# AnamarijaKic/bioinfo1

Measured on AMD Instinct MI355X. Metric: GCUPS (DP cell updates/s) at 1/2/4/8 GPUs; bit-exact score+CIGAR, higher is better.
Workload: dtype int32 semantics; packed int16 arithmetic where range-proven (fits_int16), else int32; 1 GPU; config 2: 10000 uniform 1000x1000 pairs per GPU, local, scoring 1,-1,-1, CIGAR on; pairs_per_gpu=10000, qlen=1000, tlen=1000, mode=local, cigar=True, cells_per_gpu=10000000000, cells_total=10000000000, parallelism=pairs range-split over 1 GPU(s)

## Files before the change

bioinfo1_amd/align.py:

```python
from __future__ import annotations

import ctypes as C
import enum
import os
from dataclasses import dataclass

import numpy as np

HERE = os.path.dirname(os.path.abspath(__file__))
LIB_PATH = os.path.join(HERE, "libteam_alignment.so")

TA_OK, TA_ERR_BAD_TYPE, TA_ERR_CIGAR, TA_ERR_ARG, TA_ERR_DEVICE, TA_ERR_CAPACITY, TA_ERR_RANGE, TA_ERR_UNSERVED = range(8)
TA_PLAN_INT32_ONLY, TA_PLAN_NO_FLEX, TA_PLAN_UNFUSED, TA_PLAN_WALK1, TA_PLAN_WALK2 = 1, 2, 4, 8, 16
TA_PLAN_SERIAL_PASSES, TA_PLAN_PASS_MAJOR, TA_PLAN_NO_BLK, TA_PLAN_NO_CK, TA_PLAN_CK = 32, 64, 128, 256, 512
TA_PLAN_NO_FLEX_CK = 1024


class AlignmentType(enum.IntEnum):

    global_ = 0
    local = 1
    semiGlobal = 2


class DeviceError(RuntimeError):
    pass


_lib = None


def lib() -> C.CDLL:
    global _lib
    if _lib is not None:
        return _lib
    try:
        import torch
    except ImportError:
        pass
    if not os.path.exists(LIB_PATH):
        raise ImportError(f"{LIB_PATH} missing: run `python -c 'import __graft_entry__ as g; g.build()'`")
    L = C.CDLL(LIB_PATH)
    u32p, u64p, i32p = C.POINTER(C.c_uint32), C.POINTER(C.c_uint64), C.POINTER(C.c_int32)
    L.ta_status_string.restype = C.c_char_p
    L.ta_status_string.argtypes = [C.c_int]
    L.ta_last_error.restype = C.c_char_p
    L.ta_last_error.argtypes = [C.c_void_p]
    L.ta_context_create.argtypes = [C.c_int, C.POINTER(C.c_void_p)]
    L.ta_context_destroy.argtypes = [C.c_void_p]
    L.ta_context_destroy.restype = None
    L.ta_cigar_slot_bytes.restype = C.c_uint64
    L.ta_cigar_slot_bytes.argtypes = [C.c_uint32, C.c_uint32]
    L.ta_align_batch.argtypes = [C.c_void_p, C.c_uint32, C.c_void_p, u64p, u32p, C.c_void_p, u64p, u32p, C.c_int,
                                 C.c_int, C.c_int, C.c_int, C.c_int, i32p, u32p, C.c_void_p, C.c_uint64, u64p, u32p]
    L.ta_align_batch_flags.argtypes = L.ta_align_batch.argtypes + [C.c_uint32]
    L.ta_context_release.argtypes = [C.c_void_p]
    L.ta_context_release.restype = None
    L.ta_context_held_bytes.argtypes = [C.c_void_p]
    L.ta_context_held_bytes.restype = C.c_uint64
    L.ta_set_default_device.argtypes = [C.c_int]
    L.ta_set_thread_device.argtypes = [C.c_int]
    L.ta_plan_create.argtypes = [C.c_void_p, C.c_uint32, u32p, u32p, C.c_int, C.c_int, C.c_int, C.c_int, C.c_int,
                                 C.c_uint64, C.c_uint32, C.POINTER(C.c_void_p)]
    L.ta_plan_destroy.argtypes = [C.c_void_p]
    L.ta_plan_destroy.restype = None
    for f in ("ta_plan_cigar_slots_bytes", "ta_plan_workspace_bytes"):
        getattr(L, f).restype = C.c_uint64
        getattr(L, f).argtypes = [C.c_void_p]
    L.ta_plan_chunks.restype = C.c_uint32
    L.ta_plan_chunks.argtypes = [C.c_void_p]
    L.ta_plan_dual_pairs.restype = C.c_uint32
    L.ta_plan_dual_pairs.argtypes = [C.c_void_p]
    L.ta_plan_flex_pairs.restype = C.c_uint32
    L.ta_plan_flex_pairs.argtypes = [C.c_void_p]
    L.ta_plan_fused.argtypes = [C.c_void_p]
    L.ta_plan_walk.argtypes = [C.c_void_p]
    L.ta_plan_pair_chunks.argtypes = [C.c_void_p, u32p]
    L.ta_affine_plan_pair_chunks.argtypes = [C.c_void_p, u32p]
    L.ta_plan_execute.argtypes = [C.c_void_p, C.c_void_p, C.c_void_p]
    L.ta_plan_check.argtypes = [C.c_void_p]
    L.ta_compact_cigars.argtypes = [C.c_void_p, C.c_uint32, C.c_void_p, C.c_void_p, C.c_void_p, C.c_void_p,
                                    C.c_void_p, C.c_void_p]
    L.ta_plan_execute_fill.argtypes = [C.c_void_p, C.c_void_p, C.c_void_p, C.c_uint32]
    L.ta_plan_execute_traceback.argtypes = [C.c_void_p, C.c_void_p, C.c_void_p, C.c_uint32]
    L.ta_pipeline_create.argtypes = [C.POINTER(C.c_void_p), C.c_uint32, C.POINTER(C.c_void_p)]
    L.ta_pipeline_create_affine.argtypes = L.ta_pipeline_create.argtypes
    L.ta_pipeline_step.argtypes = [C.c_void_p, C.c_void_p, C.c_void_p, C.c_void_p, u32p]
    L.ta_pipeline_destroy.argtypes = [C.c_void_p]
    L.ta_pipeline_destroy.restype = None
    L.ta_align_batch_affine.argtypes = [C.c_void_p, C.c_uint32, C.c_void_p, u64p, u32p, C.c_void_p, u64p, u32p,
                                        C.c_int, C.c_int, C.c_int, C.c_int, C.c_int, C.c_int, i32p, u32p, C.c_void_p,
                                        C.c_uint64, u64p, u32p]
    L.ta_affine_plan_create.argtypes = [C.c_void_p, C.c_uint32, u32p, u32p, C.c_int, C.c_int, C.c_int, C.c_int,
                                        C.c_int, C.c_int, C.c_uint64, C.c_uint32, C.POINTER(C.c_void_p)]
    L.ta_affine_plan_destroy.argtypes = [C.c_void_p]
    L.ta_affine_plan_destroy.restype = None
    for f in ("ta_affine_plan_cigar_slots_bytes", "ta_affine_plan_workspace_bytes"):
        getattr(L, f).restype = C.c_uint64
        getattr(L, f).argtypes = [C.c_void_p]
    L.ta_affine_plan_chunks.restype = C.c_uint32
    L.ta_affine_plan_chunks.argtypes = [C.c_void_p]
    L.ta_affine_plan_dual_pairs.restype = C.c_uint32
    L.ta_affine_plan_dual_pairs.argtypes = [C.c_void_p]
    L.ta_affine_plan_execute.argtypes = [C.c_void_p, C.c_void_p, C.c_void_p]
    L.ta_affine_plan_execute_fill.argtypes = [C.c_void_p, C.c_void_p, C.c_void_p, C.c_uint32]
    L.ta_affine_plan_execute_traceback.argtypes = [C.c_void_p, C.c_void_p, C.c_void_p, C.c_uint32]
    L.ta_affine_plan_check.argtypes = [C.c_void_p]
    L.ta_align_batch_banded.argtypes = [C.c_void_p, C.c_uint32, C.c_void_p, u64p, u32p, C.c_void_p, u64p, u32p, u32p,
                                        C.c_int, C.c_int, C.c_int, C.c_int, C.c_int, i32p, u32p, C.c_void_p,
                                        C.c_uint64, u64p, u32p]
    L.ta_banded_plan_create.argtypes = [C.c_void_p, C.c_uint32, u32p, u32p, u32p, C.c_int, C.c_int, C.c_int, C.c_int,
                                        C.c_int, C.c_uint64, C.c_uint32, C.POINTER(C.c_void_p)]
    L.ta_banded_plan_destroy.argtypes = [C.c_void_p]
    L.ta_banded_plan_destroy.restype = None
    for f in ("ta_banded_plan_cigar_slots_bytes", "ta_banded_plan_workspace_bytes", "ta_banded_plan_band_cells",
              "ta_banded_plan_swept_cells"):
        getattr(L, f).restype = C.c_uint64
        getattr(L, f).argtypes = [C.c_void_p]
    L.ta_banded_plan_chunks.restype = C.c_uint32
    L.ta_banded_plan_chunks.argtypes = [C.c_void_p]
    L.ta_banded_plan_pair_chunks.argtypes = [C.c_void_p, u32p]
    L.ta_banded_plan_execute.argtypes = [C.c_void_p, C.c_void_p, C.c_void_p]
    L.ta_banded_plan_execute_fill.argtypes = [C.c_void_p, C.c_void_p, C.c_void_p, C.c_uint32]
    L.ta_banded_plan_execute_traceback.argtypes = [C.c_void_p, C.c_void_p, C.c_void_p, C.c_uint32]
    L.ta_banded_plan_check.argtypes = [C.c_void_p]
    L.ta_banded_plan_annotate.argtypes = [C.c_void_p, C.c_void_p, C.c_void_p, C.c_void_p]
    L.ta_plan_annotate.argtypes = [C.c_void_p, C.c_void_p, C.c_void_p, C.c_void_p]
    L.ta_affine_plan_annotate.argtypes = [C.c_void_p, C.c_void_p, C.c_void_p, C.c_void_p]
    L.ta_server_create.argtypes = [C.c_int, C.c_int, C.c_uint32, C.POINTER(C.c_void_p)]
    L.ta_server_destroy.argtypes = [C.c_void_p]
    L.ta_server_destroy.restype = None
    L.ta_server_fits.argtypes = [C.c_void_p, C.c_uint32, C.c_uint32, C.c_int, C.c_int, C.c_int]
    L.ta_server_running.argtypes = [C.c_void_p]
    L.ta_server_last_times.argtypes = [C.c_void_p, C.c_uint32, C.POINTER(C.c_double)]
    L.ta_server_align.argtypes = [C.c_void_p, C.c_char_p, C.c_uint32, C.c_char_p, C.c_uint32, C.c_int, C.c_int,
                                  C.c_int, C.c_int, C.POINTER(C.c_int32), C.POINTER(C.c_uint32), C.c_void_p,
                                  C.c_uint64, C.POINTER(C.c_uint32)]
    _lib = L
    return L


ABI_SYMBOLS = [
    "ta_status_string", "ta_last_error", "ta_context_create", "ta_context_destroy", "ta_context_release",
    "ta_context_held_bytes", "ta_set_default_device", "ta_set_thread_device", "ta_current_device", "ta_device_count",
    "ta_cigar_slot_bytes", "ta_align_batch", "ta_align_batch_flags", "ta_plan_create", "ta_plan_destroy", "ta_plan_cigar_slots_bytes",
    "ta_plan_workspace_bytes", "ta_plan_chunks", "ta_plan_dual_pairs", "ta_plan_flex_pairs", "ta_plan_fused", "ta_plan_walk",
    "ta_plan_execute", "ta_plan_check", "ta_plan_execute_fill", "ta_plan_pair_chunks", "ta_affine_plan_pair_chunks", "ta_plan_execute_traceback", "ta_compact_cigars",
    "ta_affine_plan_create", "ta_affine_plan_destroy", "ta_affine_plan_cigar_slots_bytes",
    "ta_affine_plan_workspace_bytes", "ta_affine_plan_chunks", "ta_affine_plan_dual_pairs", "ta_affine_plan_execute", "ta_affine_plan_execute_fill",
    "ta_affine_plan_execute_traceback", "ta_affine_plan_check", "ta_align_batch_affine",
    "ta_server_create", "ta_server_destroy", "ta_server_fits", "ta_server_align", "ta_server_running",
    "ta_server_last_times", "ta_server_pause", "ta_server_resume",
    "ta_plan_annotate", "ta_affine_plan_annotate",
    "ta_plan_context", "ta_affine_plan_context", "ta_context_device",
    "ta_pipeline_create", "ta_pipeline_create_affine", "ta_pipeline_step", "ta_pipeline_destroy",
]
BANDED_ABI_SYMBOLS = [
    "ta_banded_plan_create", "ta_banded_plan_destroy", "ta_banded_plan_cigar_slots_bytes",
    "ta_banded_plan_workspace_bytes", "ta_banded_plan_chunks", "ta_banded_plan_pair_chunks",
    "ta_banded_plan_band_cells", "ta_banded_plan_swept_cells", "ta_banded_plan_execute",
    "ta_banded_plan_execute_fill", "ta_banded_plan_execute_traceback", "ta_banded_plan_check",
    "ta_banded_plan_annotate", "ta_align_batch_banded",
]
ABI_SYMBOLS += BANDED_ABI_SYMBOLS
TEAM_ALIGN_SYMBOL = ("_ZN4team5AlignEPKcjS1_jNS_13AlignmentTypeEiiiPNSt7__cxx1112basic_stringIcSt11char_traitsIcESaIcEEEPj")


def _check_type(type) -> int:
    t = int(type)
    if t not in (0, 1, 2):
        raise ValueError("Unknown AlignmentType provided.")
    return t


def _raise(status: int, ctx=None):
    L = lib()
    msg = L.ta_status_string(status).decode()
    if status in (TA_ERR_BAD_TYPE, TA_ERR_CIGAR, TA_ERR_RANGE):
        raise ValueError(msg)
    detail = L.ta_last_error(ctx).decode() if ctx else ""
    raise DeviceError(f"{msg}: {detail}" if detail else msg)


def _p(a, ct):
    return a.ctypes.data_as(C.POINTER(ct))


def _band_array(band, n_pairs: int) -> np.ndarray:
    if np.ndim(band) == 0:
        b = np.full(n_pairs, int(band), np.int64)
    else:
        b = np.asarray(band, np.int64).reshape(-1)
        if b.size != n_pairs:
            raise ValueError(f"band: {b.size} entries for {n_pairs} pairs")
    if b.size and (b.min() < 0 or b.max() > 0xFFFFFFFF):
        raise ValueError("band: values must be in [0, 2^32)")
    return np.ascontiguousarray(b.astype(np.uint32))


@dataclass
class BatchResult:
    scores: np.ndarray
    target_begins: np.ndarray
    cigar_offsets: np.ndarray | None
    cigar_lens: np.ndarray | None
    arena: np.ndarray | None

    def cigar(self, p: int) -> bytes | None:
        if self.arena is None:
            return None
        o = int(self.cigar_offsets[p])
        return self.arena[o : o + int(self.cigar_lens[p])].tobytes()

    def cigars(self):
        return [self.cigar(p) for p in range(len(self.scores))]


class Aligner:

    def __init__(self, device: int = 0):
        L = lib()
        h = C.c_void_p()
        r = L.ta_context_create(device, C.byref(h))
        if r != TA_OK:
            raise DeviceError(f"ta_context_create(device={device}): {L.ta_status_string(r).decode()}")
        self._h = h
        self.device = device

    def close(self):
        if getattr(self, "_h", None):
            lib().ta_context_destroy(self._h)
            self._h = None

    def __del__(self):
        try:
            self.close()
        except Exception:
            pass
# ... 316 lines not shown
            self.eqx_len = torch.zeros(self.P, dtype=torch.int32, device=self.dev)
        self._annotated_eqx = bool(eqx)
        aio = _AnnotateIO(self.info.data_ptr(), self.eqx_slots.data_ptr() if eqx else None,
                          self.eqx_start.data_ptr() if eqx else None, self.eqx_len.data_ptr() if eqx else None)
        r = self._fn("ta_plan_annotate")(self._h, C.byref(self.io), C.byref(aio), self._stream())
        if r != TA_OK:
            _raise(r, self._ctx)

    def annotation(self) -> Annotation:
        if getattr(self, "info", None) is None:
            raise RuntimeError("annotation(): no annotate() was enqueued")
        self.check()
        info = np.ascontiguousarray(self.info.cpu().numpy()).view(np.uint32).reshape(self.P, 10)
        info = info.view(PAIR_INFO_DTYPE).reshape(self.P)
        if not self._annotated_eqx:
            return Annotation(info, None, None, None)
        return Annotation(info, self.eqx_start.cpu().numpy().view(np.uint64),
                          self.eqx_len.cpu().numpy().view(np.uint32), self.eqx_slots.cpu().numpy())

    def compact_cigars(self, out=None):
        torch = self.torch
        lens = self.cigar_len.to(torch.int64)
        if out is None:
            off = torch.zeros(self.P + 1, dtype=torch.int64, device=self.dev)
            dst = torch.empty(max(self.slots_bytes, 1), dtype=torch.uint8, device=self.dev)
        else:
            dst, off = out
        torch.cumsum(lens, 0, out=off[1:])
        r = lib().ta_compact_cigars(self._ctx, self.P, self.slots.data_ptr(), self.cigar_start.data_ptr(),
                                    self.cigar_len.data_ptr(), off.data_ptr(), dst.data_ptr(), self._stream())
        if r != TA_OK:
            _raise(r, self._ctx)
        return dst, off

    def compact_buffers(self):
        torch = self.torch
        return (torch.empty(max(self.slots_bytes, 1), dtype=torch.uint8, device=self.dev),
                torch.zeros(self.P + 1, dtype=torch.int64, device=self.dev))

    def pair_chunks(self) -> np.ndarray:
        out = np.zeros(max(self.P, 1), np.uint32)
        r = self._fn("ta_plan_pair_chunks")(self._h, _p(out, C.c_uint32))
        if r != TA_OK:
            _raise(r, self._ctx)
        return out[: self.P]

    def results_at(self, indices) -> BatchResult:
        torch = self.torch
        self.check()
        idx = torch.as_tensor(np.asarray(indices, np.int64), device=self.dev)
        sc = self.score[idx].cpu().numpy()
        tb = self.target_begin[idx].cpu().numpy().view(np.uint32)
        if not self.want_cigar:
            return BatchResult(sc, tb, None, None, None)
        start = self.cigar_start[idx].cpu().numpy()
        ln = self.cigar_len[idx].cpu().numpy().view(np.uint32)
        parts, offs, o = [], np.zeros(len(ln), np.uint64), 0
        for k in range(len(ln)):
            parts.append(self.slots[int(start[k]):int(start[k]) + int(ln[k])].cpu().numpy())
            offs[k] = o
            o += int(ln[k])
        arena = np.concatenate(parts) if parts else np.zeros(1, np.uint8)
        return BatchResult(sc, tb, offs, ln, arena)

    def results(self) -> BatchResult:
        self.check()
        return _results(self)

    def close(self):
        if getattr(self, "_h", None):
            self._fn("ta_plan_destroy")(self._h)
            self._h = None

    def __del__(self):
        try:
            self.close()
        except Exception:
            pass


class DevicePipeline:

    def __init__(self, device: int, batch, type, match, mismatch, gap, want_cigar=True, depth: int = 3,
                 workspace_budget: int = 0, gap_open=None, flags: int = 0, inputs=None, first=None):
        import torch

        self.torch = torch
        self.dev = torch.device("cuda", device)
        self.aligners, self.plans, self.k = [], [], 0
        for k in range(depth):
            if k == 0 and first is not None:
                self.plans.append(first)
                continue
            al = Aligner(device)
            self.aligners.append(al)
            shared = inputs if not self.plans else (self.plans[0].qbytes, self.plans[0].qoff,
                                                    self.plans[0].tbytes, self.plans[0].toff)
            self.plans.append(DevicePlan(al, batch, type, match, mismatch, gap, want_cigar,
                                         workspace_budget=workspace_budget, gap_open=gap_open, flags=flags,
                                         inputs=shared))
        L = lib()
        handles = (C.c_void_p * len(self.plans))(*[p._h for p in self.plans])
        h = C.c_void_p()
        create = L.ta_pipeline_create_affine if self.plans[0].affine else L.ta_pipeline_create
        r = create(handles, len(self.plans), C.byref(h))
        if r != TA_OK:
            msg = L.ta_last_error(self.plans[0]._ctx).decode()
            for p in self.plans[1 if first is not None else 0:]:
                p.close()
            for al in self.aligners:
                al.close()
            if r == TA_ERR_ARG:
                raise ValueError(msg or "ta_pipeline_create: invalid argument")
            raise DeviceError(f"{L.ta_status_string(r).decode()}: {msg}")
        self._h = h

    @property
    def chunks(self):
        return self.plans[0].chunks

    def step(self, inputs=None, ready=None):
        if ready is not None and inputs is None:
            raise ValueError("DevicePipeline.step: ready without inputs (the event belongs to an upload of inputs)")
        plan = self.plans[self.k % len(self.plans)]
        if inputs is not None:
            plan.set_inputs(inputs)
        cur = self.torch.cuda.current_stream(self.dev)
        slot = C.c_uint32()
        ev = C.c_void_p(ready.cuda_event) if ready is not None else None
        r = lib().ta_pipeline_step(self._h, C.byref(plan.io), ev, C.c_void_p(cur.cuda_stream), C.byref(slot))
        if r != TA_OK:
            _raise(r, plan._ctx)
        assert self.plans[slot.value] is plan
        self.k += 1
        return plan

    def check(self):
        for p in self.plans:
            p.check()

    def close(self):
        if getattr(self, "_h", None):
            lib().ta_pipeline_destroy(self._h)
            self._h = None
        for p in self.plans:
            p.close()
        for al in self.aligners:
            al.close()


class HostBatchRunner:

    def __init__(self, aligner: Aligner, batch, type, match, mismatch, gap, want_cigar=True):
        import torch

        self.t = _check_type(type)
        self.sc = (match, mismatch, gap)
        self.want_cigar = bool(want_cigar)
        self.aligner = aligner
        self.P = P = batch.n_pairs

        def pinned(a):
            a = np.ascontiguousarray(a)
            t = torch.empty(max(a.nbytes, 1), dtype=torch.uint8, pin_memory=True)
            v = t.numpy()[: a.nbytes].view(a.dtype)
            v[...] = a.reshape(-1)
            return t, v

        self._keep = []
        for name, a in (("qb", batch.qbytes if batch.qbytes.size else np.zeros(1, np.uint8)), ("qoff", batch.qoff),
                        ("qlen", batch.qlen), ("tb", batch.tbytes if batch.tbytes.size else np.zeros(1, np.uint8)),
                        ("toff", batch.toff), ("tlen", batch.tlen), ("score", np.zeros(P, np.int32)),
                        ("tbeg", np.zeros(P, np.uint32)), ("coff", np.zeros(P, np.uint64)),
                        ("clen", np.zeros(P, np.uint32))):
            t, v = pinned(a)
            self._keep.append(t)
            setattr(self, name, v)
        cap = int((2 * (batch.qlen.astype(np.uint64) + batch.tlen.astype(np.uint64)) + 2).sum()) if P else 1
        t, self.arena = pinned(np.zeros(max(cap, 1), np.uint8))
        self._keep.append(t)
        self.cap = cap

    def run(self):
        L = lib()
        r = L.ta_align_batch(
            self.aligner.handle, self.P, self.qb.ctypes.data, _p(self.qoff, C.c_uint64), _p(self.qlen, C.c_uint32),
            self.tb.ctypes.data, _p(self.toff, C.c_uint64), _p(self.tlen, C.c_uint32), self.t, *self.sc,
            int(self.want_cigar), _p(self.score, C.c_int32), _p(self.tbeg, C.c_uint32), self.arena.ctypes.data,
            self.cap, _p(self.coff, C.c_uint64), _p(self.clen, C.c_uint32))
        if r != TA_OK:
            _raise(r, self.aligner.handle)

    def results(self) -> BatchResult:
        if not self.want_cigar:
            return BatchResult(self.score.copy(), self.tbeg.copy(), None, None, None)
        return BatchResult(self.score.copy(), self.tbeg.copy(), self.coff.copy(), self.clen.copy(), self.arena.copy())


# ... 109 lines not shown
```

bioinfo1_amd/csrc/ta_kernels.hip:

```cpp
#include <algorithm>
#include <cstdlib>

#include "ta_device.h"
#include "ta_walk2.h"
#include "ta_walk_lane.h"
#include "ta_walk_band.h"

namespace ta {
namespace {

#ifdef TA_FILL_MODE
struct PairOut {
    int score;
    uint32_t tb, gi, gj;
    uint64_t cstart;
    uint32_t clen;
};

template <int MODE>
__device__ __forceinline__ PairOut degenerate(int gap, uint32_t n, uint32_t m) {
    PairOut o{0, 0, 0, 0, 0, 0};
    if (MODE == kGlobal) {
        o.gi = n;
        o.gj = m;
// ... 722 lines not shown
                       hb = (uint32_t)rdlane((int)v, 2);
        if (seq != last) {
            __builtin_amdgcn_fence(__ATOMIC_ACQUIRE, "");
            serve_one<MODE>(sa, s, slot, seq, lane, wall_clock64(), lds);
            last = seq;
            t_hb = wall_clock64();
            continue;
        }
        if (stop) break;
        const uint64_t now = wall_clock64();
        if (hb != hb_last) {
            hb_last = hb;
            t_hb = now;
        } else if (now - t_hb > sa.hb_timeout) {
            break;
        }
        __builtin_amdgcn_s_sleep(2);
    }
}
#endif

#endif

#ifdef TA_TU_MISC
template <int MODE>
#ifndef TA_TB_WPE
#define TA_TB_WPE 8
#endif
__global__ __launch_bounds__(kBlock) __attribute__((amdgpu_waves_per_eu(TA_TB_WPE))) void traceback_kernel(TraceArgs a) {
    const int lane = threadIdx.x & 63;
    const uint32_t stride = gridDim.x * kWavesPerBlock;
    for (uint32_t widx = wave_id(); widx < a.count; widx += stride) {
        const uint32_t p = a.order ? a.order[a.begin + widx] : a.begin + widx;
        const uint32_t n = a.qlen[p], m = a.tlen[p];
        uint64_t st;
        uint32_t len;
        const WalkSeq seq{a.qbytes + a.qoff[p], a.tbytes + a.toff[p], MODE == kLocal ? a.score[p] : 0, a.match,
                          a.mismatch, a.gap};
        traceback_pair<MODE>(a.ptrs + a.ptr_off[p], n, m, a.goal_i[p], a.goal_j[p], a.slots + a.slot_off[p],
                             cigar_slot_bytes(n, m), lane, &st, &len, seq, a.blk != 0);
        if (lane == 0) {
            a.cigar_start[p] = a.slot_off[p] + st;
            a.cigar_len[p] = len;
        }
    }
}

template <int G>
__global__ __launch_bounds__(kBlock) void traceback_group_kernel(TraceArgs a) {
    const uint32_t widx = wave_id();
    if ((64u / G) * widx >= a.count) return;
    traceback_group_local<G>(a, widx, threadIdx.x & 63);
}

template <int G>
__global__ __launch_bounds__(kWave) void traceback_lane_kernel(TraceArgs a) {
    __shared__ uint32_t lds[(64 / G) * kLwGroupDw];
    traceback_lane_local<G>(a, lds, (int)threadIdx.x);
}

__global__ __launch_bounds__(kWave) __attribute__((amdgpu_waves_per_eu(1, 1))) void traceback_band_kernel(TraceArgs a) {
    __shared__ __attribute__((aligned(16))) uint8_t lds[kWave * kBwRegion + kBwStageBytes];
    const int lane = (int)threadIdx.x;
    traceback_band_local(a, lds, lane);
    if (a.fb_count) {
        const uint32_t nfb = *a.fb_count;
        for (uint32_t w = blockIdx.x; w < nfb; w += gridDim.x) {
            const uint32_t p = a.fb_order[w];
            const uint32_t n = a.qlen[p], m = a.tlen[p];
            uint64_t st;
            uint32_t len;
            const WalkSeq seq{a.qbytes + a.qoff[p], a.tbytes + a.toff[p], a.score[p], a.match, a.mismatch, a.gap};
            traceback_pair<kLocal>(a.ptrs + a.ptr_off[p], n, m, a.goal_i[p], a.goal_j[p], a.slots + a.slot_off[p],
                                   cigar_slot_bytes(n, m), lane, &st, &len, seq, true);
            if (lane == 0) {
                a.cigar_start[p] = a.slot_off[p] + st;
                a.cigar_len[p] = len;
            }
        }
    }
}

__global__ __launch_bounds__(kBlock) void format_runs_kernel(TraceArgs a) {
    const uint32_t w = wave_id();
    if (w >= a.count) return;
    format_runs(a, a.order ? a.order[a.begin + w] : a.begin + w, threadIdx.x & 63);
}

__global__ __launch_bounds__(kBlock) void compact_kernel(CompactArgs a) {
    const int lane = threadIdx.x & 63;
    const uint32_t p = wave_id();
    if (p >= a.n_pairs) return;
    const char* src = a.slots + a.cigar_start[p];
    char* dst = a.dst + a.dst_off[p];
    const uint32_t len = a.cigar_len[p];
    for (uint32_t k = (uint32_t)lane; k < len; k += 64u) dst[k] = src[k];
}

#endif

inline dim3 grid_for(uint32_t waves) { return dim3((waves + kWavesPerBlock - 1) / kWavesPerBlock); }

}

#ifdef TA_FILL_MODE
template <>
hipError_t launch_fill_mode<TA_FILL_MODE, (TA_FILL_CIGAR != 0)>(bool wide, const FillArgs& a, hipStream_t s) {
    constexpr int MODE = TA_FILL_MODE;
    constexpr bool CIGAR = TA_FILL_CIGAR != 0;
    if (!a.count) return hipSuccess;
    const dim3 g = grid_for(a.count), b(kBlock);
    if (a.count_dev && a.max_blocks) {
        const dim3 gb(std::min<uint32_t>(g.x, a.max_blocks));
        if (MODE == kLocal && wide) hipLaunchKernelGGL((fill_back_kernel<MODE, CIGAR, MODE == kLocal>), gb, b, 0, s, a);
        else hipLaunchKernelGGL((fill_back_kernel<MODE, CIGAR, false>), gb, b, 0, s, a);
        return hipGetLastError();
    }
    if (a.tasks64) {
        if (a.n_tasks) {
            const dim3 gt = grid_for(a.n_tasks);
            if (MODE == kLocal && wide) hipLaunchKernelGGL((fill_pipe_kernel<MODE, CIGAR, MODE == kLocal>), gt, b, 0, s, a);
            else hipLaunchKernelGGL((fill_pipe_kernel<MODE, CIGAR, false>), gt, b, 0, s, a);
        }
        hipLaunchKernelGGL(fill_combine_kernel<MODE>, dim3((a.count + 255) / 256), dim3(256), 0, s, a);
        return hipGetLastError();
    }
    if (MODE == kLocal && wide) hipLaunchKernelGGL((fill_kernel<MODE, CIGAR, MODE == kLocal>), g, b, 0, s, a);
    else hipLaunchKernelGGL((fill_kernel<MODE, CIGAR, false>), g, b, 0, s, a);
    return hipGetLastError();
}
#if TA_FILL_CIGAR
template <>
hipError_t launch_serve_mode<TA_FILL_MODE>(const ServeArgs& a, uint32_t slots, hipStream_t s) {
    hipLaunchKernelGGL(serve_kernel<TA_FILL_MODE>, dim3(slots), dim3(kWave), 0, s, a);
    return hipGetLastError();
}
#endif
#endif

#ifdef TA_TU_MISC
#ifndef TA_LW_G
#define TA_LW_G 16
#endif
hipError_t launch_fill(int mode, bool cigar, bool wide, const FillArgs& a, hipStream_t s) {
    switch (mode * 2 + (cigar ? 1 : 0)) {
        case 0: return launch_fill_mode<kGlobal, false>(wide, a, s);
        case 1: return launch_fill_mode<kGlobal, true>(wide, a, s);
        case 2: return launch_fill_mode<kLocal, false>(wide, a, s);
        case 3: return launch_fill_mode<kLocal, true>(wide, a, s);
        case 4: return launch_fill_mode<kSemi, false>(wide, a, s);
        case 5: return launch_fill_mode<kSemi, true>(wide, a, s);
        default: return hipErrorInvalidValue;
    }
}

hipError_t launch_dual(int mode, bool cigar, const FillArgs& a, hipStream_t s) {
    switch (mode * 2 + (cigar ? 1 : 0)) {
        case 0: return launch_dual_mode<kGlobal, false>(a, s);
        case 1: return launch_dual_mode<kGlobal, true>(a, s);
        case 2: return launch_dual_mode<kLocal, false>(a, s);
        case 3: return launch_dual_mode<kLocal, true>(a, s);
        case 4: return launch_dual_mode<kSemi, false>(a, s);
        case 5: return launch_dual_mode<kSemi, true>(a, s);
        default: return hipErrorInvalidValue;
    }
}
// ... 85 lines not shown
```

bioinfo1_amd/csrc/ta_pipeline.cpp:

```cpp
#ifndef __HIP_PLATFORM_AMD__
#define __HIP_PLATFORM_AMD__ 1
#endif
#include <hip/hip_runtime_api.h>

#include <string>
#include <vector>

#include "../../include/team_align_c.h"
#include "ta_pipeline_internal.h"

namespace {

struct Ops {
    ta_context* (*context)(const void*);
    uint32_t (*chunks)(const void*);
    int (*fill)(void*, const ta_device_io*, void*, uint32_t);
    int (*walk)(void*, const ta_device_io*, void*, uint32_t);
};

const Ops kLinear = {
    [](const void* p) { return ta_plan_context(static_cast<const ta_plan*>(p)); },
    [](const void* p) { return ta_plan_chunks(static_cast<const ta_plan*>(p)); },
    [](void* p, const ta_device_io* io, void* s, uint32_t c) {
        return ta_plan_execute_fill(static_cast<ta_plan*>(p), io, s, c);
    },
    [](void* p, const ta_device_io* io, void* s, uint32_t c) {
        return ta_plan_execute_traceback(static_cast<ta_plan*>(p), io, s, c);
    },
};

const Ops kAffine = {
    [](const void* p) { return ta_affine_plan_context(static_cast<const ta_affine_plan*>(p)); },
    [](const void* p) { return ta_affine_plan_chunks(static_cast<const ta_affine_plan*>(p)); },
    [](void* p, const ta_device_io* io, void* s, uint32_t c) {
        return ta_affine_plan_execute_fill(static_cast<ta_affine_plan*>(p), io, s, c);
    },
    [](void* p, const ta_device_io* io, void* s, uint32_t c) {
        return ta_affine_plan_execute_traceback(static_cast<ta_affine_plan*>(p), io, s, c);
    },
};

int fail(ta_context* ctx, int code, const std::string& msg) {
    ta_context_set_error(ctx, msg.c_str());
    return code;
}

#define TP_HIP(ctx, expr)                                                                     \
    do {                                                                                      \
        hipError_t e_ = (expr);                                                               \
        if (e_ != hipSuccess)                                                                 \
            return fail((ctx), TA_ERR_DEVICE, std::string(#expr) + ": " + hipGetErrorString(e_)); \
    } while (0)

}

struct ta_pipeline {
    const Ops* ops = nullptr;
    int device = 0;
    std::vector<void*> slots;
    std::vector<ta_context*> ctxs;
    std::vector<hipStream_t> fill;
    hipStream_t walk = nullptr;
    std::vector<hipEvent_t> done, walked;
    hipEvent_t start = nullptr;
    std::vector<bool> used;
    uint64_t k = 0;
    int last = -1;
};

namespace {

int create(const Ops& ops, void* const* slots, uint32_t depth, ta_pipeline** out) {
    if (!out) return TA_ERR_ARG;
    *out = nullptr;
    if (!slots || !depth || !slots[0]) return TA_ERR_ARG;
    ta_context* c0 = ops.context(slots[0]);
    if (!c0) return TA_ERR_ARG;
    if (depth < 2) return fail(c0, TA_ERR_ARG, "ta_pipeline_create: depth must be at least 2");
    for (uint32_t a = 0; a < depth; ++a) {
        ta_context* ca = slots[a] ? ops.context(slots[a]) : nullptr;
        if (!ca) return fail(c0, TA_ERR_ARG, "ta_pipeline_create: null slot");
        if (ta_context_device(ca) != ta_context_device(c0))
            return fail(c0, TA_ERR_ARG, "ta_pipeline_create: slots on different devices");
        for (uint32_t b = 0; b < a; ++b)
            if (ops.context(slots[b]) == ca)
                return fail(c0, TA_ERR_ARG, "ta_pipeline_create: two slots share a context (each needs its own workspace)");
    }
    auto* p = new ta_pipeline();
    p->ops = &ops;
    p->device = ta_context_device(c0);
    p->slots.assign(slots, slots + depth);
    for (uint32_t a = 0; a < depth; ++a) p->ctxs.push_back(ops.context(slots[a]));
    p->fill.assign(depth, nullptr);
    p->done.assign(depth, nullptr);
    p->walked.assign(depth, nullptr);
    p->used.assign(depth, false);
    *out = p;
    return TA_OK;
}

int lazy_stream(ta_context* ctx, hipStream_t& s, int priority) {
    if (s) return TA_OK;
    if (hipStreamCreateWithPriority(&s, hipStreamNonBlocking, priority) != hipSuccess) {
        s = nullptr;
        return fail(ctx, TA_ERR_DEVICE, "ta_pipeline_step: hipStreamCreateWithPriority failed");
    }
    return TA_OK;
}

int lazy_event(ta_context* ctx, hipEvent_t& e) {
    if (e) return TA_OK;
    if (hipEventCreateWithFlags(&e, hipEventDisableTiming) != hipSuccess) {
        e = nullptr;
        return fail(ctx, TA_ERR_DEVICE, "ta_pipeline_step: hipEventCreateWithFlags failed");
    }
    return TA_OK;
}

}

extern "C" {

int ta_pipeline_create(ta_plan* const* slots, uint32_t depth, ta_pipeline** out) {
    return create(kLinear, reinterpret_cast<void* const*>(slots), depth, out);
}

int ta_pipeline_create_affine(ta_affine_plan* const* slots, uint32_t depth, ta_pipeline** out) {
    return create(kAffine, reinterpret_cast<void* const*>(slots), depth, out);
}

int ta_pipeline_step(ta_pipeline* p, const ta_device_io* io, void* ready_event, void* caller_stream,
                     uint32_t* slot_out) {
    if (!p) return TA_ERR_ARG;
    const uint32_t depth = (uint32_t)p->slots.size();
    const uint32_t i = (uint32_t)(p->k % depth);
    ta_context* ctx = p->ctxs[i];
    if (!io) return fail(ctx, TA_ERR_ARG, "ta_pipeline_step: null io");
    hipStream_t cur = static_cast<hipStream_t>(caller_stream);
    TP_HIP(ctx, hipSetDevice(p->device));
    if (!p->walk) {
        int least = 0, greatest = 0;
        TP_HIP(ctx, hipDeviceGetStreamPriorityRange(&least, &greatest));
        if (int r = lazy_stream(ctx, p->walk, greatest)) return r;
    }
    if (int r = lazy_stream(ctx, p->fill[i], 0)) return r;
    if (int r = lazy_event(ctx, p->done[i])) return r;
    if (int r = lazy_event(ctx, p->walked[i])) return r;
    if (!p->start) {
        if (int r = lazy_event(ctx, p->start)) return r;
        TP_HIP(ctx, hipEventRecord(p->start, cur));
    }
    if (p->last >= 0) TP_HIP(ctx, hipEventRecord(p->done[p->last], cur));
    if (slot_out) *slot_out = i;
    void* plan = p->slots[i];
    TP_HIP(ctx, hipStreamWaitEvent(p->fill[i], p->used[i] ? p->done[i] : p->start, 0));
    if (ready_event) TP_HIP(ctx, hipStreamWaitEvent(p->fill[i], static_cast<hipEvent_t>(ready_event), 0));
    const uint32_t chunks = p->ops->chunks(plan);
    for (uint32_t c = 0; c < chunks; ++c) {
        if (int r = p->ops->fill(plan, io, p->fill[i], c)) return r;
        if (int r = p->ops->walk(plan, io, p->walk, c)) return r;
    }
    TP_HIP(ctx, hipEventRecord(p->walked[i], p->walk));
    TP_HIP(ctx, hipStreamWaitEvent(cur, p->walked[i], 0));
    p->used[i] = true;
    p->last = (int)i;
    ++p->k;
    return TA_OK;
}

void ta_pipeline_destroy(ta_pipeline* p) {
    if (!p) return;
    (void)hipSetDevice(p->device);
    for (hipStream_t s : p->fill)
        if (s) (void)hipStreamDestroy(s);
    if (p->walk) (void)hipStreamDestroy(p->walk);
    for (hipEvent_t e : p->done)
        if (e) (void)hipEventDestroy(e);
    for (hipEvent_t e : p->walked)
        if (e) (void)hipEventDestroy(e);
    if (p->start) (void)hipEventDestroy(p->start);
    delete p;
}

}
```

include/team_align_c.h:

```cpp
#ifndef TEAM_ALIGN_C_H
#define TEAM_ALIGN_C_H

#include <stddef.h>
#include <stdint.h>

#ifdef __cplusplus
extern "C" {
#endif

#define TA_GLOBAL 0
#define TA_LOCAL 1
#define TA_SEMI_GLOBAL 2

#define TA_OK 0
#define TA_ERR_BAD_TYPE 1
#define TA_ERR_CIGAR 2
#define TA_ERR_ARG 3
#define TA_ERR_DEVICE 4
#define TA_ERR_CAPACITY 5

typedef struct ta_context ta_context;
typedef struct ta_plan ta_plan;

const char* ta_status_string(int status);
// ... 9 lines not shown
int ta_server_create(int device, int type, uint32_t slots, ta_server** out);
void ta_server_destroy(ta_server* server);
int ta_server_fits(const ta_server* server, uint32_t query_len, uint32_t target_len, int match, int mismatch,
                   int gap);
int ta_server_align(ta_server* server, const char* query, uint32_t query_len, const char* target,
                    uint32_t target_len, int match, int mismatch, int gap, int want_cigar, int32_t* score,
                    uint32_t* target_begin, char* cigar, uint64_t cigar_capacity, uint32_t* cigar_len);
int ta_server_running(const ta_server* server);
int ta_server_pause(ta_server* server);
int ta_server_resume(ta_server* server);
int ta_server_last_times(const ta_server* server, uint32_t slot, double* us_out4);

int ta_set_default_device(int device);
int ta_set_thread_device(int device);
int ta_current_device(void);
int ta_device_count(void);

uint64_t ta_cigar_slot_bytes(uint32_t query_len, uint32_t target_len);

int ta_align_batch(ta_context* ctx, uint32_t n_pairs, const char* query_bytes, const uint64_t* query_off,
                   const uint32_t* query_len, const char* target_bytes, const uint64_t* target_off,
                   const uint32_t* target_len, int type, int match, int mismatch, int gap, int want_cigar,
                   int32_t* score, uint32_t* target_begin, char* cigar_arena, uint64_t cigar_arena_bytes,
                   uint64_t* cigar_off, uint32_t* cigar_len);

int ta_align_batch_flags(ta_context* ctx, uint32_t n_pairs, const char* query_bytes, const uint64_t* query_off,
                         const uint32_t* query_len, const char* target_bytes, const uint64_t* target_off,
                         const uint32_t* target_len, int type, int match, int mismatch, int gap, int want_cigar,
                         int32_t* score, uint32_t* target_begin, char* cigar_arena, uint64_t cigar_arena_bytes,
                         uint64_t* cigar_off, uint32_t* cigar_len, uint32_t flags);

#define TA_PLAN_INT32_ONLY 1u
#define TA_PLAN_NO_FLEX 2u
#define TA_PLAN_UNFUSED 4u
#define TA_PLAN_WALK1 8u
#define TA_PLAN_WALK2 16u
#define TA_PLAN_SERIAL_PASSES 32u
#define TA_PLAN_PASS_MAJOR 64u
#define TA_PLAN_NO_BLK 128u
#define TA_PLAN_NO_CK 256u
#define TA_PLAN_CK 512u
#define TA_PLAN_NO_FLEX_CK 1024u
int ta_plan_create(ta_context* ctx, uint32_t n_pairs, const uint32_t* query_len_host,
                   const uint32_t* target_len_host, int type, int match, int mismatch, int gap, int want_cigar,
                   uint64_t workspace_budget, uint32_t flags, ta_plan** out);
void ta_plan_destroy(ta_plan* plan);
uint64_t ta_plan_cigar_slots_bytes(const ta_plan* plan);
uint64_t ta_plan_workspace_bytes(const ta_plan* plan);
uint32_t ta_plan_chunks(const ta_plan* plan);
uint32_t ta_plan_dual_pairs(const ta_plan* plan);
uint32_t ta_plan_flex_pairs(const ta_plan* plan);
int ta_plan_fused(const ta_plan* plan);
int ta_plan_walk(const ta_plan* plan);
int ta_plan_pair_chunks(const ta_plan* plan, uint32_t* chunk_of_pair);

typedef struct ta_device_io {
    const char* query_bytes;
    const uint64_t* query_off;
    const char* target_bytes;
    const uint64_t* target_off;
    int32_t* score;
    uint32_t* target_begin;
    char* cigar_slots;
    uint64_t* cigar_start;
    uint32_t* cigar_len;
} ta_device_io;

int ta_plan_execute(ta_plan* plan, const ta_device_io* io, void* hip_stream);

int ta_plan_check(ta_plan* plan);

int ta_plan_execute_fill(ta_plan* plan, const ta_device_io* io, void* hip_stream, uint32_t chunk);
int ta_plan_execute_traceback(ta_plan* plan, const ta_device_io* io, void* hip_stream, uint32_t chunk);

ta_context* ta_plan_context(const ta_plan* plan);
int ta_context_device(const ta_context* ctx);

typedef struct ta_pipeline ta_pipeline;
int ta_pipeline_create(ta_plan* const* slots, uint32_t depth, ta_pipeline** out);
int ta_pipeline_step(ta_pipeline* pipe, const ta_device_io* io, void* ready_event, void* caller_stream,
                     uint32_t* slot_out);
void ta_pipeline_destroy(ta_pipeline* pipe);

int ta_compact_cigars(ta_context* ctx, uint32_t n_pairs, const char* cigar_slots, const uint64_t* cigar_start,
                      const uint32_t* cigar_len, const uint64_t* dst_off, char* dst, void* hip_stream);

typedef struct ta_pair_info {
    uint32_t query_begin, query_end;
    uint32_t target_begin, target_end;
    uint32_t n_eq, n_x, n_ins, n_del;
    uint32_t n_gap_runs;
    uint32_t n_free;
} ta_pair_info;

typedef struct ta_annotate_io {
    ta_pair_info* info;
    char* eqx_slots;
    uint64_t* eqx_start;
    uint32_t* eqx_len;
} ta_annotate_io;

int ta_plan_annotate(ta_plan* plan, const ta_device_io* io, const ta_annotate_io* out, void* hip_stream);

#define TA_ERR_RANGE 6
#define TA_ERR_UNSERVED 7

typedef struct ta_affine_plan ta_affine_plan;

int ta_affine_plan_create(ta_context* ctx, uint32_t n_pairs, const uint32_t* query_len_host,
                          const uint32_t* target_len_host, int type, int match, int mismatch, int gap_open,
                          int gap_extend, int want_cigar, uint64_t workspace_budget, uint32_t flags,
                          ta_affine_plan** out);
void ta_affine_plan_destroy(ta_affine_plan* plan);
uint64_t ta_affine_plan_cigar_slots_bytes(const ta_affine_plan* plan);
uint64_t ta_affine_plan_workspace_bytes(const ta_affine_plan* plan);
uint32_t ta_affine_plan_chunks(const ta_affine_plan* plan);
uint32_t ta_affine_plan_dual_pairs(const ta_affine_plan* plan);
int ta_affine_plan_pair_chunks(const ta_affine_plan* plan, uint32_t* chunk_of_pair);
int ta_affine_plan_execute(ta_affine_plan* plan, const ta_device_io* io, void* hip_stream);
int ta_affine_plan_execute_fill(ta_affine_plan* plan, const ta_device_io* io, void* hip_stream, uint32_t chunk);
int ta_affine_plan_execute_traceback(ta_affine_plan* plan, const ta_device_io* io, void* hip_stream,
                                     uint32_t chunk);
int ta_affine_plan_check(ta_affine_plan* plan);
ta_context* ta_affine_plan_context(const ta_affine_plan* plan);
int ta_pipeline_create_affine(ta_affine_plan* const* slots, uint32_t depth, ta_pipeline** out);
int ta_affine_plan_annotate(ta_affine_plan* plan, const ta_device_io* io, const ta_annotate_io* out,
                            void* hip_stream);

int ta_align_batch_affine(ta_context* ctx, uint32_t n_pairs, const char* query_bytes, const uint64_t* query_off,
                          const uint32_t* query_len, const char* target_bytes, const uint64_t* target_off,
                          const uint32_t* target_len, int type, int match, int mismatch, int gap_open,
                          int gap_extend, int want_cigar, int32_t* score, uint32_t* target_begin,
                          char* cigar_arena, uint64_t cigar_arena_bytes, uint64_t* cigar_off, uint32_t* cigar_len);

typedef struct ta_banded_plan ta_banded_plan;

int ta_banded_plan_create(ta_context* ctx, uint32_t n_pairs, const uint32_t* query_len_host,
                          const uint32_t* target_len_host, const uint32_t* band_host, int type, int match,
                          int mismatch, int gap, int want_cigar, uint64_t workspace_budget, uint32_t flags,
                          ta_banded_plan** out);
void ta_banded_plan_destroy(ta_banded_plan* plan);
uint64_t ta_banded_plan_cigar_slots_bytes(const ta_banded_plan* plan);
uint64_t ta_banded_plan_workspace_bytes(const ta_banded_plan* plan);
uint32_t ta_banded_plan_chunks(const ta_banded_plan* plan);
int ta_banded_plan_pair_chunks(const ta_banded_plan* plan, uint32_t* chunk_of_pair);
uint64_t ta_banded_plan_band_cells(const ta_banded_plan* plan);
uint64_t ta_banded_plan_swept_cells(const ta_banded_plan* plan);
int ta_banded_plan_execute(ta_banded_plan* plan, const ta_device_io* io, void* hip_stream);
int ta_banded_plan_execute_fill(ta_banded_plan* plan, const ta_device_io* io, void* hip_stream, uint32_t chunk);
int ta_banded_plan_execute_traceback(ta_banded_plan* plan, const ta_device_io* io, void* hip_stream,
                                     uint32_t chunk);
int ta_banded_plan_check(ta_banded_plan* plan);
int ta_banded_plan_annotate(ta_banded_plan* plan, const ta_device_io* io, const ta_annotate_io* out,
                            void* hip_stream);

int ta_align_batch_banded(ta_context* ctx, uint32_t n_pairs, const char* query_bytes, const uint64_t* query_off,
                          const uint32_t* query_len, const char* target_bytes, const uint64_t* target_off,
                          const uint32_t* target_len, const uint32_t* band, int type, int match, int mismatch,
                          int gap, int want_cigar, int32_t* score, uint32_t* target_begin, char* cigar_arena,
                          uint64_t cigar_arena_bytes, uint64_t* cigar_off, uint32_t* cigar_len);

#ifdef __cplusplus
}
#endif

#endif
```

Baseline: 8035 GCUPS.

## Allow multiple high-priority traceback streams in pipeline and raise format kernel priority

After: 8405 GCUPS, median of 6. 1.05x the previous value.

```diff
diff --git a/bioinfo1_amd/align.py b/bioinfo1_amd/align.py
--- a/bioinfo1_amd/align.py
+++ b/bioinfo1_amd/align.py
@@ -85,6 +85,10 @@
     L.ta_plan_execute_traceback.argtypes = [C.c_void_p, C.c_void_p, C.c_void_p, C.c_uint32]
     L.ta_pipeline_create.argtypes = [C.POINTER(C.c_void_p), C.c_uint32, C.POINTER(C.c_void_p)]
     L.ta_pipeline_create_affine.argtypes = L.ta_pipeline_create.argtypes
+    L.ta_pipeline_create_ex.argtypes = [C.POINTER(C.c_void_p), C.c_uint32, C.c_void_p, C.POINTER(C.c_void_p)]
+    L.ta_pipeline_create_affine_ex.argtypes = L.ta_pipeline_create_ex.argtypes
+    L.ta_pipeline_walk_streams.argtypes = [C.c_void_p]
+    L.ta_pipeline_walk_streams.restype = C.c_uint32
     L.ta_pipeline_step.argtypes = [C.c_void_p, C.c_void_p, C.c_void_p, C.c_void_p, u32p]
     L.ta_pipeline_destroy.argtypes = [C.c_void_p]
     L.ta_pipeline_destroy.restype = None
@@ -154,6 +158,7 @@
     "ta_plan_annotate", "ta_affine_plan_annotate",
     "ta_plan_context", "ta_affine_plan_context", "ta_context_device",
     "ta_pipeline_create", "ta_pipeline_create_affine", "ta_pipeline_step", "ta_pipeline_destroy",
+    "ta_pipeline_create_ex", "ta_pipeline_create_affine_ex", "ta_pipeline_walk_streams",
 ]
 BANDED_ABI_SYMBOLS = [
     "ta_banded_plan_create", "ta_banded_plan_destroy", "ta_banded_plan_cigar_slots_bytes",
@@ -636,7 +641,8 @@
 class DevicePipeline:
 
     def __init__(self, device: int, batch, type, match, mismatch, gap, want_cigar=True, depth: int = 3,
-                 workspace_budget: int = 0, gap_open=None, flags: int = 0, inputs=None, first=None):
+                 workspace_budget: int = 0, gap_open=None, flags: int = 0, inputs=None, first=None,
+                 walk_streams=None):
         import torch
 
         self.torch = torch
@@ -656,8 +662,9 @@
         L = lib()
         handles = (C.c_void_p * len(self.plans))(*[p._h for p in self.plans])
         h = C.c_void_p()
-        create = L.ta_pipeline_create_affine if self.plans[0].affine else L.ta_pipeline_create
-        r = create(handles, len(self.plans), C.byref(h))
+        create = L.ta_pipeline_create_affine_ex if self.plans[0].affine else L.ta_pipeline_create_ex
+        opts = (C.c_uint32 * 2)(8, int(walk_streams or 0))
+        r = create(handles, len(self.plans), opts, C.byref(h))
         if r != TA_OK:
             msg = L.ta_last_error(self.plans[0]._ctx).decode()
             for p in self.plans[1 if first is not None else 0:]:
@@ -668,6 +675,7 @@
                 raise ValueError(msg or "ta_pipeline_create: invalid argument")
             raise DeviceError(f"{L.ta_status_string(r).decode()}: {msg}")
         self._h = h
+        self.walk_streams = L.ta_pipeline_walk_streams(h)
 
     @property
     def chunks(self):
diff --git a/bioinfo1_amd/csrc/ta_kernels.hip b/bioinfo1_amd/csrc/ta_kernels.hip
--- a/bioinfo1_amd/csrc/ta_kernels.hip
+++ b/bioinfo1_amd/csrc/ta_kernels.hip
@@ -828,6 +828,7 @@
 }
 
 __global__ __launch_bounds__(kBlock) void format_runs_kernel(TraceArgs a) {
+    __builtin_amdgcn_s_setprio(3);
     const uint32_t w = wave_id();
     if (w >= a.count) return;
     format_runs(a, a.order ? a.order[a.begin + w] : a.begin + w, threadIdx.x & 63);
diff --git a/bioinfo1_amd/csrc/ta_pipeline.cpp b/bioinfo1_amd/csrc/ta_pipeline.cpp
--- a/bioinfo1_amd/csrc/ta_pipeline.cpp
+++ b/bioinfo1_amd/csrc/ta_pipeline.cpp
@@ -3,6 +3,8 @@
 #endif
 #include <hip/hip_runtime_api.h>
 
+#include <cstddef>
+#include <cstdlib>
 #include <string>
 #include <vector>
 
@@ -60,7 +62,7 @@
     std::vector<void*> slots;
     std::vector<ta_context*> ctxs;
     std::vector<hipStream_t> fill;
-    hipStream_t walk = nullptr;
+    std::vector<hipStream_t> walk;
     std::vector<hipEvent_t> done, walked;
     hipEvent_t start = nullptr;
     std::vector<bool> used;
@@ -70,7 +72,21 @@
 
 namespace {
 
-int create(const Ops& ops, void* const* slots, uint32_t depth, ta_pipeline** out) {
+uint32_t hw_queues() {
+    const char* v = std::getenv("GPU_MAX_HW_QUEUES");
+    if (!v || !*v) return 4;
+    char* end = nullptr;
+    const long n = std::strtol(v, &end, 10);
+    return (*end || n <= 0) ? 4u : (uint32_t)n;
+}
+
+uint32_t resolve_walk_streams(uint32_t asked, uint32_t depth) {
+    if (asked) return asked;
+    const uint32_t w = TA_PIPELINE_WALK_STREAMS_DEFAULT < depth ? TA_PIPELINE_WALK_STREAMS_DEFAULT : depth;
+    return hw_queues() >= depth + w + 1 ? w : 1;
+}
+
+int create(const Ops& ops, void* const* slots, uint32_t depth, const ta_pipeline_options* opt, ta_pipeline** out) {
     if (!out) return TA_ERR_ARG;
     *out = nullptr;
     if (!slots || !depth || !slots[0]) return TA_ERR_ARG;
@@ -86,12 +102,21 @@
             if (ops.context(slots[b]) == ca)
                 return fail(c0, TA_ERR_ARG, "ta_pipeline_create: two slots share a context (each needs its own workspace)");
     }
+    uint32_t w = 1;
+    if (opt) {
+        const bool has = opt->size >= offsetof(ta_pipeline_options, walk_streams) + sizeof(opt->walk_streams);
+        w = resolve_walk_streams(has ? opt->walk_streams : 0, depth);
+    }
+    if (w > depth)
+        return fail(c0, TA_ERR_ARG, "ta_pipeline_create: walk_streams exceeds depth (" + std::to_string(w) + " > " +
+                                        std::to_string(depth) + ")");
     auto* p = new ta_pipeline();
     p->ops = &ops;
     p->device = ta_context_device(c0);
     p->slots.assign(slots, slots + depth);
     for (uint32_t a = 0; a < depth; ++a) p->ctxs.push_back(ops.context(slots[a]));
     p->fill.assign(depth, nullptr);
+    p->walk.assign(w, nullptr);
     p->done.assign(depth, nullptr);
     p->walked.assign(depth, nullptr);
     p->used.assign(depth, false);
@@ -122,12 +147,26 @@
 extern "C" {
 
 int ta_pipeline_create(ta_plan* const* slots, uint32_t depth, ta_pipeline** out) {
-    return create(kLinear, reinterpret_cast<void* const*>(slots), depth, out);
+    return create(kLinear, reinterpret_cast<void* const*>(slots), depth, nullptr, out);
+}
+
+int ta_pipeline_create_ex(ta_plan* const* slots, uint32_t depth, const ta_pipeline_options* options,
+                          ta_pipeline** out) {
+    const ta_pipeline_options defaults = {sizeof(ta_pipeline_options), 0};
+    return create(kLinear, reinterpret_cast<void* const*>(slots), depth, options ? options : &defaults, out);
 }
 
 int ta_pipeline_create_affine(ta_affine_plan* const* slots, uint32_t depth, ta_pipeline** out) {
-    return create(kAffine, reinterpret_cast<void* const*>(slots), depth, out);
-}
+    return create(kAffine, reinterpret_cast<void* const*>(slots), depth, nullptr, out);
+}
+
+int ta_pipeline_create_affine_ex(ta_affine_plan* const* slots, uint32_t depth, const ta_pipeline_options* options,
+                                 ta_pipeline** out) {
+    const ta_pipeline_options defaults = {sizeof(ta_pipeline_options), 0};
+    return create(kAffine, reinterpret_cast<void* const*>(slots), depth, options ? options : &defaults, out);
+}
+
+uint32_t ta_pipeline_walk_streams(const ta_pipeline* p) { return p ? (uint32_t)p->walk.size() : 0; }
 
 int ta_pipeline_step(ta_pipeline* p, const ta_device_io* io, void* ready_event, void* caller_stream,
                      uint32_t* slot_out) {
@@ -138,11 +177,13 @@
     if (!io) return fail(ctx, TA_ERR_ARG, "ta_pipeline_step: null io");
     hipStream_t cur = static_cast<hipStream_t>(caller_stream);
     TP_HIP(ctx, hipSetDevice(p->device));
-    if (!p->walk) {
+    if (!p->walk.back()) {
         int least = 0, greatest = 0;
         TP_HIP(ctx, hipDeviceGetStreamPriorityRange(&least, &greatest));
-        if (int r = lazy_stream(ctx, p->walk, greatest)) return r;
-    }
+        for (hipStream_t& s : p->walk)
+            if (int r = lazy_stream(ctx, s, greatest)) return r;
+    }
+    hipStream_t walk = p->walk[p->k % p->walk.size()];
     if (int r = lazy_stream(ctx, p->fill[i], 0)) return r;
     if (int r = lazy_event(ctx, p->done[i])) return r;
     if (int r = lazy_event(ctx, p->walked[i])) return r;
@@ -158,9 +199,9 @@
     const uint32_t chunks = p->ops->chunks(plan);
     for (uint32_t c = 0; c < chunks; ++c) {
         if (int r = p->ops->fill(plan, io, p->fill[i], c)) return r;
-        if (int r = p->ops->walk(plan, io, p->walk, c)) return r;
-    }
-    TP_HIP(ctx, hipEventRecord(p->walked[i], p->walk));
+        if (int r = p->ops->walk(plan, io, walk, c)) return r;
+    }
+    TP_HIP(ctx, hipEventRecord(p->walked[i], walk));
     TP_HIP(ctx, hipStreamWaitEvent(cur, p->walked[i], 0));
     p->used[i] = true;
     p->last = (int)i;
@@ -173,7 +214,8 @@
     (void)hipSetDevice(p->device);
     for (hipStream_t s : p->fill)
         if (s) (void)hipStreamDestroy(s);
-    if (p->walk) (void)hipStreamDestroy(p->walk);
+    for (hipStream_t s : p->walk)
+        if (s) (void)hipStreamDestroy(s);
     for (hipEvent_t e : p->done)
         if (e) (void)hipEventDestroy(e);
     for (hipEvent_t e : p->walked)
diff --git a/include/team_align_c.h b/include/team_align_c.h
--- a/include/team_align_c.h
+++ b/include/team_align_c.h
@@ -115,6 +115,17 @@
                      uint32_t* slot_out);
 void ta_pipeline_destroy(ta_pipeline* pipe);
 
+#ifndef TA_PIPELINE_WALK_STREAMS_DEFAULT
+#define TA_PIPELINE_WALK_STREAMS_DEFAULT 1u
+#endif
+typedef struct ta_pipeline_options {
+    uint32_t size;
+    uint32_t walk_streams;
+} ta_pipeline_options;
+int ta_pipeline_create_ex(ta_plan* const* slots, uint32_t depth, const ta_pipeline_options* options,
+                          ta_pipeline** out);
+uint32_t ta_pipeline_walk_streams(const ta_pipeline* pipe);
+
 int ta_compact_cigars(ta_context* ctx, uint32_t n_pairs, const char* cigar_slots, const uint64_t* cigar_start,
                       const uint32_t* cigar_len, const uint64_t* dst_off, char* dst, void* hip_stream);
 
@@ -157,6 +168,8 @@
 int ta_affine_plan_check(ta_affine_plan* plan);
 ta_context* ta_affine_plan_context(const ta_affine_plan* plan);
 int ta_pipeline_create_affine(ta_affine_plan* const* slots, uint32_t depth, ta_pipeline** out);
+int ta_pipeline_create_affine_ex(ta_affine_plan* const* slots, uint32_t depth, const ta_pipeline_options* options,
+                                 ta_pipeline** out);
 int ta_affine_plan_annotate(ta_affine_plan* plan, const ta_device_io* io, const ta_annotate_io* out,
                             void* hip_stream);
 
```
